# IceTTTb/NopeSAC

Measured on AMD Instinct MI355X. Metric: image-pairs/sec (480x640, K=32 hyp), higher is better.
Workload: dtype bf16; 1 GPU; configs/inference_mp3d.yaml, 32 synthetic 480x640 pairs/GPU/step, ResNet-50 + pyramids in bfloat16, head GEMMs bf16 operands with f32 accumulate / residual stream / LayerNorm / softmax, K=32 matched planes forced (m mean 32.0), nq=50; pairs_per_gpu=32, global_batch=32, K=32, parallelism=pair-sharded dp1, rccl_ranks=1, batches_in_flight_per_gpu=4, hip_graph=False, steps_per_all_gather=8, routing_entries_loaded=45, routing_entries_measured_now=0, nonfinite_outputs=0

## Files before the change

include/nopesac_hip.h:

```cpp
#ifndef NOPESAC_HIP_H
#define NOPESAC_HIP_H

#include <stdint.h>

#ifdef __cplusplus
extern "C" {
#endif

#define NPS_DT_F32 0
#define NPS_DT_BF16 1
#define NPS_DT_F32_BF16W 2
#define NPS_DT_FP8 3

#define NPS_ACT_NONE 0
#define NPS_ACT_RELU 1
#define NPS_ACT_LEAKY 2
#define NPS_ACT_SIGMOID 3
#define NPS_ACT_RES_AFTER 0x100
#define NPS_ACT_BIAS_BATCHED 0x200

#define NPS_E_ARG (-1)
#define NPS_E_UNSUPPORTED (-2)
typedef int nps_status;

// ... 248 lines not shown
nps_status nopesac_force_k_select(const float* logits, int n_cls, const float* query_feat, const int64_t* perm, const float* noise,
                                  int B, int nq, int K, int D, float* feats, int32_t* n_kept, void* stream);

nps_status nopesac_normalize_rows(const float* x, float* y, int rows, int D, int canonical_sign, void* stream);

nps_status nopesac_count_nonfinite(const float* x, int64_t n, int32_t* count, void* stream);
nps_status nopesac_u8_to_f32(const uint8_t* x, float* y, int64_t n, void* stream);

nps_status nopesac_clock_probe(uint64_t* out2, int64_t spin_cycles, void* stream);

#define NOPESAC_NONFINITE_MAX_TENSORS 16
nps_status nopesac_count_nonfinite_batch(const float* const* x, const int64_t* n, int n_tensors, int32_t* count, void* stream);

#define NOPESAC_JPEG_HUFF_BYTES 1536
#define NOPESAC_JPEG_TABLES_BYTES (4 * NOPESAC_JPEG_HUFF_BYTES + 3 * 128)
#define NOPESAC_JPEG_IMG_I32 32
#define NOPESAC_JPEG_IMG_I64 8
#define NOPESAC_JPEG_SEG_I32 4
#define NOPESAC_JPEG_SEG_I64 2
nps_status nopesac_jpeg_huffman(const int32_t* img32, const int64_t* img64, const uint8_t* tables, const int32_t* seg32, const int64_t* seg64,
                                int n_segments, const uint32_t* words, int64_t n_words, int16_t* coef, const int32_t* par_done, void* stream);
int64_t nopesac_jpeg_prepare_scan(const uint8_t* data, int64_t n, int has_restart, uint32_t* words, int64_t words_cap, int64_t* seg_off,
                                  int64_t* seg_cnt, int64_t* seg_bytes, int64_t max_segs, int64_t* consumed);
void* nopesac_jpeg_batch_scan_host(const char* const* paths, int n, int threads, int parallel, int* status, int64_t* totals);
int nopesac_jpeg_batch_fill_host(void* batch, int32_t* img32, int64_t* img64, uint8_t* tables, int32_t* seg32, int64_t* seg64, uint32_t* words,
                                 int32_t* lane_img, int32_t* geometry);
void nopesac_jpeg_batch_free_host(void* batch);
#define NOPESAC_JPEG_SUB_WORDS 64
#define NOPESAC_JPEG_SYNC_PASSES 12
nps_status nopesac_jpeg_huffman_parallel(const int32_t* img32, const int64_t* img64, const uint8_t* tables, int n_images, const int32_t* lane_img,
                                         int64_t n_lanes, const uint32_t* words, int64_t n_words, int64_t* exit_state, int64_t* entry_used,
                                         int32_t* n_blk, int64_t* first_block, int32_t* changed, int32_t* par_done, int16_t* coef, void* stream);
nps_status nopesac_jpeg_idct(const int32_t* img32, const int64_t* img64, const uint8_t* tables, int n_images, int n_blocks, const int16_t* coef,
                             uint8_t* planes, void* stream);
nps_status nopesac_jpeg_color(const int32_t* img32, const int64_t* img64, int n_images, int max_pixels, const uint8_t* planes, uint8_t* out,
                              int bgr, void* stream);

#define NOPESAC_GATHER_MAX_SEGMENTS 32
nps_status nopesac_gather_bytes(const void* const* src, const int64_t* size, const int64_t* const* size_dev, const int64_t* dst_off,
                                int n_segments, void* dst, void* stream);

nps_status nopesac_gnn_layer_bf16(const float* x, int x_off, const float* src, int src_off, float* out, int out_off, int n_sets, int nq,
                                  const int32_t* qlen, const int32_t* klen, const void* wq, const void* wk, const void* wv,
                                  const void* wmerge, const void* w0, const void* w2, const float* ln1_g, const float* ln1_b,
                                  const float* ln2_g, const float* ln2_b, void* stream);
nps_status nopesac_gnn_layer_bf16_pf(const float* x, int x_off, const float* src, int src_off, float* out, int out_off, int n_sets,
                                     int nq, const int32_t* qlen, const int32_t* klen, const void* wq, const void* wk, const void* wv,
                                     const void* wmerge, const void* w0, const void* w2, const float* ln1_g, const float* ln1_b,
                                     const float* ln2_g, const float* ln2_b, const void* const* next_weights6, int next_sets, void* stream);

nps_status nopesac_mask_head_bf16(const void* c1, const void* t1, const void* w_lateral, const float* scale, const float* bias,
                                  const void* mask_w, const float* mask_b, float* prob, void* p1_out, int B, int H, int W, int nq,
                                  int apply_sigmoid, void* stream);

nps_status nopesac_mask_operands(const float* fold, int ld, void* mask_w, float* mask_b, int B, int nq, int nqp, void* stream);

nps_status nopesac_encoder_tail_bf16(const void* attn, const float* src, const void* wo, const float* bo, const float* ln1_g,
                                     const float* ln1_b, const void* w1, const float* b1, const void* w2, const float* b2,
                                     const float* ln2_g, const float* ln2_b, const float* pos, int pos_rows, float* y, void* y_bf16,
                                     void* ypos_bf16, int M, void* stream);

nps_status nopesac_resize_bilinear_u8(const uint8_t* src, int H, int W, int C, uint8_t* dst, int OH, int OW, void* stream);
nps_status nopesac_resize_bilinear_u8_batch(const uint8_t* src, int n, int64_t src_stride, int H, int W, int C, uint8_t* dst, int OH, int OW, int chw,
                                            void* stream);

nps_status nopesac_decoder_tail_bf16(const void* attn, const float* tgt, const void* wo, const float* bo, const float* ln3_g,
                                     const float* ln3_b, const void* w1, const float* b1, const void* w2, const float* b2,
                                     const float* lnn_g, const float* lnn_b, const float* pos, int pos_rows, float* y, void* y_bf16,
                                     void* ypos_bf16, float* yn, int M, void* stream);

nps_status nopesac_transformer_tail_bf16(const void* attn, const float* src, const void* wo, const float* bo, const float* lna_g,
                                         const float* lna_b, const void* w1, const float* b1, const void* w2, const float* b2,
                                         const float* lnb_g, const float* lnb_b, const float* pos, int pos_rows, float* y, void* y_bf16,
                                         void* ypos_bf16, float* yn, int pre_norm, int skip_ffn, const void* w_pos, const float* b_pos,
                                         void* proj_pos, int n_pos, const void* w_proj, const float* b_proj, void* proj, int n_proj, int M,
                                         void* stream);
nps_status nopesac_transformer_tail_bf16_pf(const void* attn, const float* src, const void* wo, const float* bo, const float* lna_g,
                                            const float* lna_b, const void* w1, const float* b1, const void* w2, const float* b2,
                                            const float* lnb_g, const float* lnb_b, const float* pos, int pos_rows, float* y, void* y_bf16,
                                            void* ypos_bf16, float* yn, int pre_norm, int skip_ffn, const void* w_pos, const float* b_pos,
                                            void* proj_pos, int n_pos, const void* w_proj, const float* b_proj, void* proj, int n_proj, int M,
                                            const void* const* next_ptrs, const int64_t* next_bytes, int n_next, int next_workgroups, void* stream);

#define NPS_ETAIL_32 0
#define NPS_ETAIL_64 1
#define NPS_ETAIL_96 2
#define NPS_ETAIL_128 3
#define NPS_ETAIL_FORMS 4
#define NPS_ETAIL_SW_32 1
#define NPS_ETAIL_SW_64 2
#define NPS_ETAIL_SW_ROWS 4
#define NPS_ETAIL_SW_ROWS3 8
int nopesac_transformer_tail_forms(long long M, int pre_norm, int skip_ffn, long long n_proj_total, int switches, unsigned* eligible);
nps_status nopesac_transformer_tail_bf16_form(const void* attn, const float* src, const void* wo, const float* bo, const float* lna_g,
                                              const float* lna_b, const void* w1, const float* b1, const void* w2, const float* b2,
                                              const float* lnb_g, const float* lnb_b, const float* pos, int pos_rows, float* y, void* y_bf16,
                                              void* ypos_bf16, float* yn, int pre_norm, int skip_ffn, const void* w_pos, const float* b_pos,
                                              void* proj_pos, int n_pos, const void* w_proj, const float* b_proj, void* proj, int n_proj, int M,
                                              const void* const* next_ptrs, const int64_t* next_bytes, int n_next, int next_workgroups, int form,
                                              void* stream);

nps_status nopesac_rle_labels(const uint8_t* winner, const int32_t* kept_idx, const int32_t* n_kept, const int32_t* flags,
                              uint8_t* labels, int V, int H, int W, int nq, void* stream);
nps_status nopesac_rle_transitions(const uint8_t* labels, const int32_t* n_kept, const int64_t* offsets, int32_t* counts,
                                   uint32_t* positions, int V, int N, int nq, void* stream);
nps_status nopesac_decode_masks(const uint8_t* winner, const int32_t* kept_idx, const int32_t* n_kept, const int32_t* flags,
// ... 158 lines not shown
```

nopesac_amd/build.py:

```python
from __future__ import annotations

import hashlib
import os
import shutil
import subprocess
import sys
from concurrent.futures import ThreadPoolExecutor

HERE = os.path.dirname(os.path.abspath(__file__))
CSRC = os.path.join(HERE, "csrc")
LIB = os.path.join(HERE, "libnopesac_hip.so")
OBJ = os.path.join(CSRC, "_obj")
SOURCES = ["capi.hip", "conv_igemm.hip", "conv_p8.hip", "conv_p8n.hip", "stem.hip", "conv3x3_c64.hip", "conv3x3_halo.hip", "pwchain.hip", "gnn_layer.hip", "enc_tail.hip", "mask_head.hip", "resize.hip", "rle.hip", "plane_eval.hip", "elementwise.hip", "attention.hip", "postselect.hip", "matcher.hip",
           "ransac.hip", "refine_bwd.hip", "conv_bwd.hip", "matcher_bwd.hip", "plane_criterion.hip", "mlp_chain.hip", "tape.hip", "posenet_branch.hip", "jpeg.hip", "jpeg_host.hip", "png_host.hip"]
FLAGS = ["--offload-arch=gfx950", "-O3", "-std=c++17", "-fPIC", "-ffp-contract=off", "-Xclang", "-target-feature", "-Xclang", "-packed-fp32-ops"]
if os.environ.get("NOPESAC_ALLOW_PACKED_FP32"):
    FLAGS = FLAGS[:5]
EXTRA_FLAGS = {}
if os.environ.get("NOPESAC_HIPCC_EXTRA"):
    FLAGS = FLAGS + os.environ["NOPESAC_HIPCC_EXTRA"].split()


def _hipcc() -> str:
    for c in (os.environ.get("HIPCC"), shutil.which("hipcc"), "/opt/rocm/bin/hipcc"):
        if c and os.path.exists(c):
            return c
    raise RuntimeError("hipcc not found (need ROCm with gfx950 support)")


def _have_zlib(cc: str) -> bool:
    import tempfile
    with tempfile.TemporaryDirectory() as d:
        src = os.path.join(d, "z.cpp")
        with open(src, "w") as f:
            f.write("#include <zlib.h>\nint main() { z_stream s{}; return inflateInit(&s) == Z_OK ? inflateEnd(&s) : 1; }\n")
        r = subprocess.run([cc, "-x", "c++", src, "-o", os.path.join(d, "z"), "-lz"], capture_output=True, text=True)
        return r.returncode == 0


def _digest() -> str:
    h = hashlib.sha256((" ".join(FLAGS) + repr(sorted(EXTRA_FLAGS.items()))).encode())
    for name in sorted(os.listdir(CSRC)) + ["../../include/nopesac_hip.h"]:
        p = os.path.join(CSRC, name)
        if os.path.isfile(p) and (name.endswith((".hip", ".h"))):
            h.update(name.encode())
            h.update(open(p, "rb").read())
    return h.hexdigest()


def build(force: bool = False, verbose: bool = True) -> str:
    stamp = os.path.join(OBJ, "digest.txt")
    dig = _digest()
    if not force and os.path.exists(LIB) and os.path.exists(stamp) and open(stamp).read() == dig:
        return LIB
    os.makedirs(OBJ, exist_ok=True)
    cc = _hipcc()
    have_zlib = _have_zlib(cc)
    per_build = {"png_host.hip": ["-DNPS_HAVE_ZLIB=%d" % int(have_zlib)]}

    def compile_one(src):
        obj = os.path.join(OBJ, src.replace(".hip", ".o"))
        cmd = [cc, *FLAGS, *EXTRA_FLAGS.get(src, []), *per_build.get(src, []), "-c", os.path.join(CSRC, src), "-o", obj]
        r = subprocess.run(cmd, capture_output=True, text=True)
        if r.returncode != 0:
            raise RuntimeError("hipcc failed on %s:\n%s" % (src, r.stderr[-4000:]))
        return obj
# ... 17 lines not shown
```

nopesac_amd/csrc/common.h:

```cpp
#pragma once
#include <hip/hip_runtime.h>
#include <stdint.h>
#include <stdio.h>
#include <string.h>

#include <atomic>

#include "../../include/nopesac_hip.h"

namespace nps {

typedef unsigned short bf16_t;

__device__ __forceinline__ float bf16_to_f32(bf16_t v) { return __uint_as_float(((uint32_t)v) << 16); }
__device__ __forceinline__ bf16_t f32_to_bf16(float f) { return __builtin_bit_cast(bf16_t, (__bf16)f); }
__device__ __forceinline__ uint32_t f32x2_to_bf16x2(float lo, float hi) {
    typedef float f32x2_t __attribute__((ext_vector_type(2)));
    typedef __bf16 bf16x2_t __attribute__((ext_vector_type(2)));
    const f32x2_t v = {lo, hi};
    return __builtin_bit_cast(uint32_t, __builtin_convertvector(v, bf16x2_t));
}

__device__ __forceinline__ uint2 f32x8_to_fp8(const float* v) {
    float c[8];
// ... 5 lines not shown
    hi = __builtin_amdgcn_cvt_pk_fp8_f32(c[4], c[5], hi, false);
    hi = __builtin_amdgcn_cvt_pk_fp8_f32(c[6], c[7], hi, true);
    return make_uint2((unsigned)lo, (unsigned)hi);
}

template <typename T> __device__ __forceinline__ float to_f32(T v);
template <> __device__ __forceinline__ float to_f32<float>(float v) { return v; }
template <> __device__ __forceinline__ float to_f32<bf16_t>(bf16_t v) { return bf16_to_f32(v); }
template <typename T> __device__ __forceinline__ T from_f32(float v);
template <> __device__ __forceinline__ float from_f32<float>(float v) { return v; }
template <> __device__ __forceinline__ bf16_t from_f32<bf16_t>(float v) { return f32_to_bf16(v); }

__device__ __forceinline__ float apply_act(float v, int act) {
    if (act == NPS_ACT_SIGMOID) return 1.f / (1.f + expf(-v));
    const float neg = act == NPS_ACT_RELU ? 0.f : (act == NPS_ACT_LEAKY ? 0.01f * v : v);
    return v > 0.f ? v : neg;
}

template <int N>
__device__ __forceinline__ void apply_act_n(float (&v)[N], int act) {
    if (act == NPS_ACT_RELU) {
#pragma unroll
        for (int e = 0; e < N; ++e) v[e] = v[e] > 0.f ? v[e] : 0.f;
    } else if (act == NPS_ACT_LEAKY) {
#pragma unroll
        for (int e = 0; e < N; ++e) v[e] = v[e] > 0.f ? v[e] : 0.01f * v[e];
    } else if (act == NPS_ACT_SIGMOID) {
#pragma unroll
        for (int e = 0; e < N; ++e) v[e] = 1.f / (1.f + expf(-v[e]));
    }
}

__device__ __forceinline__ void act_residual8(float (&v)[8], const float (&r)[8], int act, int res_after) {
    if (!res_after) {
#pragma unroll
        for (int e = 0; e < 8; ++e) v[e] += r[e];
    }
    if (act == NPS_ACT_RELU) {
#pragma unroll
        for (int e = 0; e < 8; ++e) v[e] = v[e] > 0.f ? v[e] : 0.f;
    } else if (act == NPS_ACT_LEAKY) {
#pragma unroll
        for (int e = 0; e < 8; ++e) v[e] = v[e] > 0.f ? v[e] : 0.01f * v[e];
    } else if (act == NPS_ACT_SIGMOID) {
#pragma unroll
        for (int e = 0; e < 8; ++e) v[e] = 1.f / (1.f + expf(-v[e]));
    }
    if (res_after) {
#pragma unroll
        for (int e = 0; e < 8; ++e) v[e] += r[e];
    }
}

__device__ __forceinline__ float wave_sum(float v) {
#pragma unroll
    for (int o = 32; o > 0; o >>= 1) v += __shfl_xor(v, o, 64);
    return v;
}
__device__ __forceinline__ float wave_max(float v) {
#pragma unroll
    for (int o = 32; o > 0; o >>= 1) v = fmaxf(v, __shfl_xor(v, o, 64));
    return v;
}

__device__ __forceinline__ void quat_to_rot(const float q[4], float R[9]) {
    const float w = q[0], x = q[1], y = q[2], z = q[3];
    R[0] = 1 - 2 * y * y - 2 * z * z; R[1] = 2 * x * y - 2 * w * z; R[2] = 2 * x * z + 2 * w * y;
    R[3] = 2 * x * y + 2 * w * z; R[4] = 1 - 2 * x * x - 2 * z * z; R[5] = 2 * y * z - 2 * w * x;
    R[6] = 2 * x * z - 2 * w * y; R[7] = 2 * y * z + 2 * w * x; R[8] = 1 - 2 * x * x - 2 * y * y;
}

__device__ __forceinline__ void warp_plane(const float p[3], const float R[9], const float t[3], float out[3]) {
    const float f0 = p[0], f1 = -p[1], f2 = -p[2];
    float e[3], b[3];
#pragma unroll
    for (int i = 0; i < 3; ++i) {
        float s = __fmul_rn(R[3 * i], f0);
        s = __fmaf_rn(R[3 * i + 1], f1, s);
        s = __fmaf_rn(R[3 * i + 2], f2, s);
        e[i] = __fadd_rn(s, t[i]);
        b[i] = __fsub_rn(e[i], t[i]);
    }
    const float dot = e[0] * b[0] + e[1] * b[1] + e[2] * b[2];
    const float nb = sqrtf(b[0] * b[0] + b[1] * b[1] + b[2] * b[2]) + 1e-5f;
    const float c = dot / (nb * nb);
    out[0] = c * b[0]; out[1] = c * b[1]; out[2] = c * b[2];
}

__device__ __forceinline__ float norm3(const float v[3]) { return sqrtf(v[0] * v[0] + v[1] * v[1] + v[2] * v[2]); }
__device__ __forceinline__ void normalize3(const float v[3], float o[3]) {
    const float n = fmaxf(norm3(v), 1e-12f);
    o[0] = v[0] / n; o[1] = v[1] / n; o[2] = v[2] / n;
}

void set_error(const char* fmt, ...);

}

#define NPS_CHECK_ARG(cond, ...)               \
    do {                                       \
        if (!(cond)) {                         \
            nps::set_error(__VA_ARGS__);       \
            return NPS_E_ARG;                  \
        }                                      \
    } while (0)

// ... 22 lines not shown
```

nopesac_amd/csrc/elementwise.hip:

```cpp
#include <algorithm>

#include "common.h"

namespace nps {

template <typename T>
__global__ void preprocess_kernel(const float* __restrict__ x, T* __restrict__ y, const float* __restrict__ mean,
                                  const float* __restrict__ stdv, int B, int C, int H, int W, int Cpad) {
    const long long npix = (long long)B * H * W;
    for (long long i = blockIdx.x * (long long)blockDim.x + threadIdx.x; i < npix; i += (long long)gridDim.x * blockDim.x) {
        const long long b = i / ((long long)H * W), hw = i % ((long long)H * W);
        for (int c = 0; c < Cpad; ++c) {
            float v = 0.f;
            if (c < C) v = (x[(b * C + c) * H * W + hw] - mean[c]) / stdv[c];
            y[i * Cpad + c] = from_f32<T>(v);
        }
    }
}

template <typename T, int V> struct Pack { T v[V]; };
template <typename T, int V> __device__ __forceinline__ void load_vec(const T* p, float out[V]) {
    if constexpr (V == 1) { out[0] = to_f32<T>(*p); }
    else {
        typedef Pack<T, V> __attribute__((aligned(sizeof(T) * V))) PV;
// ... 5 lines not shown
template <typename T, int V> __device__ __forceinline__ void store_vec(T* p, const float in[V]) {
    if constexpr (V == 1) { *p = from_f32<T>(in[0]); }
    else {
        typedef Pack<T, V> __attribute__((aligned(sizeof(T) * V))) PV;
        PV pk;
#pragma unroll
        for (int i = 0; i < V; ++i) pk.v[i] = from_f32<T>(in[i]);
        *reinterpret_cast<PV*>(p) = pk;
    }
}

template <typename T, int V>
__global__ void maxpool_kernel(const T* __restrict__ x, T* __restrict__ y, int B, int H, int W, int C, int K,
                               int stride, int pad, int OH, int OW) {
    const int CV = C / V;
    const long long total = (long long)B * OH * OW * CV;
    for (long long i = blockIdx.x * (long long)blockDim.x + threadIdx.x; i < total; i += (long long)gridDim.x * blockDim.x) {
        const int c = (int)(i % CV) * V;
        long long pix = i / CV;
        const int ow = pix % OW; pix /= OW;
        const int oh = pix % OH;
        const int b = pix / OH;
        float m[V];
#pragma unroll
        for (int e = 0; e < V; ++e) m[e] = -INFINITY;
        for (int kh = 0; kh < K; ++kh) {
            const int ih = oh * stride - pad + kh;
            if ((unsigned)ih >= (unsigned)H) continue;
            for (int kw = 0; kw < K; ++kw) {
                const int iw = ow * stride - pad + kw;
                if ((unsigned)iw >= (unsigned)W) continue;
                float t[V];
                load_vec<T, V>(x + (((long long)b * H + ih) * W + iw) * C + c, t);
#pragma unroll
                for (int e = 0; e < V; ++e) m[e] = fmaxf(m[e], t[e]);
            }
        }
        store_vec<T, V>(y + (i / CV) * C + c, m);
    }
}

template <typename T, int V>
__global__ void upsample_bilinear2x_kernel(const T* __restrict__ x, const T* __restrict__ addend, T* __restrict__ y,
                                           int B, int H, int W, int C, int act) {
    const int OH = 2 * H, OW = 2 * W, CV = C / V;
    const long long total = (long long)B * OH * OW * CV;
    for (long long i = blockIdx.x * (long long)blockDim.x + threadIdx.x; i < total; i += (long long)gridDim.x * blockDim.x) {
        const int c = (int)(i % CV) * V;
        long long pix = i / CV;
        const long long opix = pix;
        const int ow = pix % OW; pix /= OW;
        const int oh = pix % OH;
        const int b = pix / OH;
        float sy = fmaxf(0.5f * (oh + 0.5f) - 0.5f, 0.f), sx = fmaxf(0.5f * (ow + 0.5f) - 0.5f, 0.f);
        const int y0 = (int)sy, x0 = (int)sx;
        const int y1 = min(y0 + 1, H - 1), x1 = min(x0 + 1, W - 1);
        const float ly = sy - y0, lx = sx - x0, hy = 1.f - ly, hx = 1.f - lx;
        const long long base = (long long)b * H * W;
        float v00[V], v01[V], v10[V], v11[V], o[V];
        load_vec<T, V>(x + (base + (long long)y0 * W + x0) * C + c, v00);
        load_vec<T, V>(x + (base + (long long)y0 * W + x1) * C + c, v01);
        load_vec<T, V>(x + (base + (long long)y1 * W + x0) * C + c, v10);
        load_vec<T, V>(x + (base + (long long)y1 * W + x1) * C + c, v11);
#pragma unroll
        for (int e = 0; e < V; ++e) o[e] = hy * (hx * v00[e] + lx * v01[e]) + ly * (hx * v10[e] + lx * v11[e]);
        apply_act_n<V>(o, act);
        if (addend) {
            float a[V];
            load_vec<T, V>(addend + opix * C + c, a);
#pragma unroll
            for (int e = 0; e < V; ++e) o[e] += a[e];
        }
        store_vec<T, V>(y + opix * C + c, o);
    }
}

template <typename T, int V>
__global__ void upsample_nearest2x_add_kernel(const T* __restrict__ x, const T* __restrict__ lat, T* __restrict__ y,
                                              int B, int H, int W, int C) {
    const int OH = 2 * H, OW = 2 * W, CV = C / V;
    const long long total = (long long)B * OH * OW * CV;
    for (long long i = blockIdx.x * (long long)blockDim.x + threadIdx.x; i < total; i += (long long)gridDim.x * blockDim.x) {
        const int c = (int)(i % CV) * V;
        long long pix = i / CV;
        const long long opix = pix;
        const int ow = pix % OW; pix /= OW;
        const int oh = pix % OH;
        const int b = pix / OH;
        float a[V], l[V];
        load_vec<T, V>(x + (((long long)b * H + (oh >> 1)) * W + (ow >> 1)) * C + c, a);
        load_vec<T, V>(lat + opix * C + c, l);
#pragma unroll
        for (int e = 0; e < V; ++e) a[e] += l[e];
        store_vec<T, V>(y + opix * C + c, a);
    }
}

template <typename T>
__global__ __launch_bounds__(256) void groupnorm_kernel(const T* __restrict__ x, const float* __restrict__ gamma,
                                                        const float* __restrict__ beta, T* __restrict__ y, int HW,
                                                        int C, int G, float eps, int act, int groups_per_block) {
    const int cpg = C / G;
    const int CPB = cpg * groups_per_block;
    const int b = blockIdx.y, chunk = blockIdx.x;
    const int c_local = threadIdx.x % CPB, prow = threadIdx.x / CPB, nprow = 256 / CPB;
    const int c = chunk * CPB + c_local;
    const int g_local = c_local / cpg;
    const T* xb = x + (long long)b * HW * C;
    T* yb = y + (long long)b * HW * C;
    __shared__ float red[256];
    __shared__ float stat[64];
    const float cnt = (float)HW * cpg;
    float s = 0.f;
    for (int p = prow; p < HW; p += nprow) s += to_f32<T>(xb[(long long)p * C + c]);
    red[threadIdx.x] = s;
    __syncthreads();
    if (threadIdx.x < groups_per_block) {
        float t = 0.f;
// ... 649 lines not shown
```

nopesac_amd/modeling/plane_head.py:

```python
from __future__ import annotations

import os

import math

import torch

from .. import _lib, ops
from ..registry import SEM_SEG_HEADS_REGISTRY
from ..synth import state_dict_spec
from .params import ConvW, ParamModule, conv_bias, conv_bn, mlp_layers


def sine_position_embedding(h: int, w: int, num_pos_feats: int = 128) -> torch.Tensor:
    eps, scale, temperature = 1e-6, 2 * math.pi, 10000.0
    y = torch.arange(1, h + 1, dtype=torch.float32).view(h, 1).expand(h, w)
    x = torch.arange(1, w + 1, dtype=torch.float32).view(1, w).expand(h, w)
    y = y / (y[-1:, :] + eps) * scale
    x = x / (x[:, -1:] + eps) * scale
    dim_t = torch.arange(num_pos_feats, dtype=torch.float32)
    dim_t = temperature ** (2 * torch.div(dim_t, 2, rounding_mode="floor") / num_pos_feats)
    px, py = x[:, :, None] / dim_t, y[:, :, None] / dim_t
    px = torch.stack((px[..., 0::2].sin(), px[..., 1::2].cos()), dim=3).flatten(2)
    py = torch.stack((py[..., 0::2].sin(), py[..., 1::2].cos()), dim=3).flatten(2)
# ... 19 lines not shown
    flat, last_of, restarts = [], [], []
    for si, (layers, final_act, out) in enumerate(stacks):
        for i, l in enumerate(layers):
            last = i == len(layers) - 1
            flat.append((l, final_act if last else ops.ACT_RELU))
            last_of.append(si if last else -1)
            restarts.append(par[si] and si > 0 and i == 0)
    want = [o for (_, _, o) in stacks]
    for si in range(len(stacks)):
        if want[si] is None and (si == len(stacks) - 1 or par[si + 1]):
            want[si] = True
    results = [None] * len(stacks)
    for si, o in enumerate(want):
        if o is True:
            results[si] = torch.empty(rows, stacks[si][0][-1].cout, device=x.device, dtype=torch.float32)
        elif o is not None:
            results[si] = o
    k0 = x.shape[1] + (0 if x_bcast is None else x_bcast.shape[1])
    few_rows = rows <= CHAIN_MIN_ROWS and sum(l.cout * l.cin for l, _ in flat) >= CHAIN_SMALL_PARAMS
    if (gd == torch.bfloat16 and x.dtype == torch.float32 and len(flat) <= _lib.MLP_MAX_LAYERS and k0 <= _lib.MLP_MAX_IN
            and all(l.cout <= _lib.MLP_MAX_WIDTH for l, _ in flat) and not few_rows):
        ops.mlp_chain(x, [l.chain() for l, _ in flat], [a for _, a in flat], [results[si] if si >= 0 else None for si in last_of],
                      x_bcast=x_bcast, rows_per=rows_per, restarts=restarts)
        return results
    if x_bcast is not None:
        assert rows == x_bcast.shape[0] * rows_per, "run_stacks: x_bcast rows x rows_per must equal the rows of x"
        full = torch.empty(rows, k0, device=x.device, dtype=torch.float32)
        full.view(-1, rows_per, k0)[:, :, :x_bcast.shape[1]] = x_bcast[:, None, :]
        full[:, x_bcast.shape[1]:] = x
        x = full
    x_in = x
    for (l, a), si, rs in zip(flat, last_of, restarts):
        inner = gd == torch.bfloat16 and (si < 0 or results[si] is None)
        x = ops.linear(x_in if rs else x, l.w2d(gd), l.bias, act=a, out=results[si] if si >= 0 else None,
                       out_dtype=torch.bfloat16 if inner else None)
    return results


@SEM_SEG_HEADS_REGISTRY.register()
class PlaneTRHead(ParamModule):
    def __init__(self, cfg, input_shape=None):
        H = cfg.MODEL.SEM_SEG_HEAD
        self.num_queries = H.NUM_OBJECT_QUERIES
        self.nheads = H.NHEADS
        assert H.HIDDEN_DIM == 256 and H.MASK_DIM == 256 and H.NHEADS == 8 and H.ENC_LAYERS == 6 and H.DEC_LAYERS == 6, \
            "PlaneTRHead kernels are specialised to hidden 256 / 8 heads / 6+6 layers (config/config.py:46-51)"
        assert H.PARAM_ON and H.CENTER_ON and not cfg.MODEL.DEPTH_ON, "inference configs set PARAM_ON/CENTER_ON, no depth"
        spec = {k[len("sem_seg_head."):]: v for k, v in state_dict_spec(self.num_queries).items()
                if k.startswith("sem_seg_head.")}
        super().__init__(spec)
        self._pos_cache = {}
        self.fused_encoder_tail = True
        self.fused_mask_head = True
        self.fused_decoder_tail = True
        self.chain_projections = True

    def _mha(self, prefix: str, fuse_qk: bool):
        w, b = self.raw(prefix + ".in_proj_weight").float(), self.raw(prefix + ".in_proj_bias").float()
        E = 256
        d = {"o": conv_bias(self, prefix + ".out_proj"), "v": ConvW(w[2 * E:], None, b[2 * E:])}
        if fuse_qk:
            d["qk"] = ConvW(w[:2 * E], None, b[:2 * E])
        else:
            d["q"], d["k"] = ConvW(w[:E], None, b[:E]), ConvW(w[E:2 * E], None, b[E:2 * E])
        return d

    def pack(self) -> dict:
        P = {"input_proj": conv_bias(self, "input_proj")}
        for i in range(6):
            p = f"context_SA.layers.{i}"
            P[p] = {"attn": self._mha(p + ".self_attn", True), "l1": conv_bias(self, p + ".linear1"),
                    "l2": conv_bias(self, p + ".linear2")}
            p = f"context2plane_decoder.layers.{i}"
            P[p] = {"self": self._mha(p + ".self_attn", True), "cross": self._mha(p + ".multihead_attn", False),
                    "l1": conv_bias(self, p + ".linear1"), "l2": conv_bias(self, p + ".linear2")}
        wk = [self.raw(f"context2plane_decoder.layers.{i}.multihead_attn.in_proj_weight").float()[256:512] for i in range(6)]
        bk = [self.raw(f"context2plane_decoder.layers.{i}.multihead_attn.in_proj_bias").float()[256:512] for i in range(6)]
        wv = [self.raw(f"context2plane_decoder.layers.{i}.multihead_attn.in_proj_weight").float()[512:768] for i in range(6)]
        bv = [self.raw(f"context2plane_decoder.layers.{i}.multihead_attn.in_proj_bias").float()[512:768] for i in range(6)]
        P["cross_k_all"] = ConvW(torch.cat(wk, 0), None, torch.cat(bk, 0))
        P["cross_v_all"] = ConvW(torch.cat(wv, 0), None, torch.cat(bv, 0))
        for nm in ("up_conv3", "up_conv2", "up_conv1", "c4_conv", "c3_conv", "c2_conv", "c1_conv", "m_conv_dict.m4"):
            P[nm] = conv_bn(self, f"top_down.{nm}.0.weight", f"top_down.{nm}.1", 1e-5)
        for nm in ("plane_embedding", "plane_param", "plane_center"):
            P[nm] = mlp_layers(self, nm)
        P["pixel_embedding"] = conv_bias(self, "pixel_embedding")
        w_pe = self.raw("pixel_embedding.weight").float().reshape(256, 256)
        fold = torch.zeros(264, 256, device=w_pe.device)
        fold[:256] = w_pe.t()
        fold[256] = self.raw("pixel_embedding.bias").float()
        P["pe_fold"] = ConvW(fold)
        P["pixel_plane_center"] = conv_bias(self, "pixel_plane_center")
        P["plane_prob"] = conv_bias(self, "plane_prob")
        return P

    def _ln(self, x, prefix, **kw):
        return ops.layernorm(x, self.raw(prefix + ".weight"), self.raw(prefix + ".bias"), **kw)

    def _pos(self, h, w, device):
        key = (h, w, str(device))
        if key not in self._pos_cache:
            self._pos_cache[key] = sine_position_embedding(h, w).to(device)
        return self._pos_cache[key]

    def forward(self, features: dict, want_logits: bool = False):
        P, gd = self.packed, self.gemm_dtype
# ... 157 lines not shown
                    hs = r["yn"]
                continue
            tgt = lin(o, W["cross"]["o"].w2d(bf), W["cross"]["o"].bias, residual=tgt, out_dtype=f32)
            r = ln(tgt, p + ".norm3", want=("y16",))
            hdn = lin(r["y16"], W["l1"].w2d(bf), W["l1"].bias, act=ops.ACT_RELU, out_dtype=bf)
            tgt = lin(hdn, W["l2"].w2d(bf), W["l2"].bias, residual=tgt, out_dtype=f32)
            if i < 5:
                nin = ln(tgt, nxt, addend=qpos, want=("y16", "y2_16"))
                n16, npos16 = nin["y16"], nin["y2_16"]
        if hs is None:
            hs = self._ln(tgt, "context2plane_decoder.norm")
        return hs, memory

    def _tail_weights(self, kind: str, i: int) -> dict:
        cache = self.__dict__.setdefault("_tail_w", {})
        if (kind, i) not in cache:
            bf = torch.bfloat16
            f = lambda k: self.raw(k).float().contiguous()
            if kind == "enc":
                e = self._enc_tail_weights(i)
                cache[(kind, i)] = dict(e, ga=e["g1"], bea=e["be1"], gb=e["g2"], beb=e["be2"])
            elif kind == "dec":
                d = self._dec_tail_weights(i, f"context2plane_decoder.layers.{i + 1}.norm1" if i < 5 else "context2plane_decoder.norm")
                cache[(kind, i)] = dict(d, ga=d["g3"], bea=d["be3"], gb=d["gn"], beb=d["ben"])
            else:
                p, W = f"context2plane_decoder.layers.{i}", self.packed[f"context2plane_decoder.layers.{i}"]
                cache[(kind, i)] = {"wo": W["self"]["o"].wfrag(bf), "bo": W["self"]["o"].bias, "ga": f(p + ".norm2.weight"), "bea": f(p + ".norm2.bias")}
        return cache[(kind, i)]

    def _dec_tail_weights(self, i: int, next_norm: str) -> dict:
        cache = self.__dict__.setdefault("_dec_tail_w", {})
        if i not in cache:
            p, W = f"context2plane_decoder.layers.{i}", self.packed[f"context2plane_decoder.layers.{i}"]
            f = lambda k: self.raw(k).float().contiguous()
            cache[i] = {"wo": W["cross"]["o"].wfrag(torch.bfloat16), "bo": W["cross"]["o"].bias, "w1": W["l1"].wfrag(torch.bfloat16),
                        "b1": W["l1"].bias, "w2": W["l2"].wfrag(torch.bfloat16), "b2": W["l2"].bias,
                        "g3": f(p + ".norm3.weight"), "be3": f(p + ".norm3.bias"),
                        "gn": f(next_norm + ".weight"), "ben": f(next_norm + ".bias")}
        return cache[i]

    def _heads(self, features, hs, memory, B, hc, wc, nq, want_logits, mark):
        P, gd = self.packed, self.gemm_dtype
        c1, c2, c3, c4 = features["res2"], features["res3"], features["res4"], features["res5"]
        cd = c4.dtype
        RA = ops.ACT_RELU | ops.ACT_RES_AFTER

        def cbr(x, nm, residual=None, out_dtype=None):
            c = P[nm]
            return ops.conv2d(x, c.w(gd if x.dtype == torch.float32 else x.dtype), c.scale, c.bias, residual,
                              act=RA if residual is not None else ops.ACT_RELU, out_dtype=out_dtype)

        p4 = cbr(memory.view(B, hc, wc, 256), "m_conv_dict.m4", residual=cbr(c4, "c4_conv"), out_dtype=cd)

        def up_stage(x, nm, lateral):
            c = P[nm]
            t = ops.conv2d(x, c.w(x.dtype), c.scale, c.bias, act=ops.ACT_NONE)
            return ops.upsample2x_bilinear(t, lateral, act=ops.ACT_RELU)

        p3 = up_stage(p4, "up_conv3", cbr(c3, "c3_conv"))
        p2 = up_stage(p3, "up_conv2", cbr(c2, "c2_conv"))
        if gd == torch.bfloat16 and hs.dtype == torch.float32:
            r = run_stacks(hs, [(P["plane_embedding"], ops.ACT_NONE, None), ([P["pe_fold"]], ops.ACT_NONE, True),
                                ([P["plane_prob"]], ops.ACT_NONE, True), (P["plane_param"], ops.ACT_NONE, True),
                                (P["plane_center"], ops.ACT_SIGMOID, True)], gd, parallel=[False, False, True, True, True])
            fold = r[1]
            heads = {"pred_logits": r[2].view(B, nq, 2), "pred_params": r[3].view(B, nq, 3), "pred_centers": r[4].view(B, nq, 2)}
        else:
            fold = run_stacks(hs, [(P["plane_embedding"], ops.ACT_NONE, None), ([P["pe_fold"]], ops.ACT_NONE, True)], gd)[1]
            heads = {
                "pred_logits": run_mlp(hs, [P["plane_prob"]], gd=gd).view(B, nq, 2),
                "pred_params": run_mlp(hs, P["plane_param"], gd=gd).view(B, nq, 3),
                "pred_centers": run_mlp(hs, P["plane_center"], final_act=ops.ACT_SIGMOID, gd=gd).view(B, nq, 2),
            }
        h1, w1 = c1.shape[1], c1.shape[2]
        if (self.fused_mask_head and cd == torch.bfloat16 and not want_logits and nq <= 128 and nq % 2 == 0 and (h1 * w1) % 128 == 0):
            c = P["up_conv1"]
            t1 = ops.conv2d(p2, c.w(cd), c.scale, c.bias, act=ops.ACT_NONE)
            l = P["c1_conv"]
            mark("ph.top_down")
            heads["mask_prob"] = ops.mask_head(c1, t1, l.wfrag(cd), l.scale, l.bias, None, None, fold=fold)
            return heads, hs.view(B, nq, 256)
        p1 = up_stage(p2, "up_conv1", cbr(c1, "c1_conv"))
        mark("ph.top_down")
        mw = fold[:, :256].to(cd).contiguous().view(B, nq, 1, 1, 256)
        mb = fold[:, 256].contiguous().view(B, nq)
        out = dict(heads)
        out["mask_prob"] = ops.conv2d(p1, mw, None, mb, batched_weights=True, act=ops.ACT_SIGMOID, out_dtype=torch.float32)
        if want_logits:
            out["pred_mask_logits"] = ops.conv2d(p1, mw, None, mb, batched_weights=True, out_dtype=torch.float32)
            pc = P["pixel_plane_center"]
            out["pixel_centers"] = ops.conv2d(p1, pc.w(cd), None, pc.bias, act=ops.ACT_SIGMOID, out_dtype=torch.float32)
        return out, hs.view(B, nq, 256)


def build_planeTR_head(cfg, input_shape=None):
    return SEM_SEG_HEADS_REGISTRY.get(cfg.MODEL.SEM_SEG_HEAD.NAME)(cfg, input_shape)


def post_select(head_out: dict, query_feat: torch.Tensor, height: int, width: int, cfg) -> dict:
    return ops.postselect_planes(head_out["pred_logits"], head_out["mask_prob"], head_out["pred_params"], query_feat,
                                 height, width, float(cfg.TEST.PLANE_SCORE_THRESHOLD), float(cfg.TEST.MASK_PROB_THRESHOLD),
                                 float(cfg.TEST.OVERLAP_THRESHOLD), planar=bool(head_out.get("mask_prob_planar", False)))
```

nopesac_amd/ops.py:

```python
from __future__ import annotations

from collections import namedtuple
from typing import Optional

import ctypes
import functools
import os

import torch

from . import _lib

_H = _lib.H
F32, BF16, FP8 = _H.NPS_DT_F32, _H.NPS_DT_BF16, _H.NPS_DT_FP8
ACT_NONE, ACT_RELU, ACT_LEAKY, ACT_SIGMOID = _H.NPS_ACT_NONE, _H.NPS_ACT_RELU, _H.NPS_ACT_LEAKY, _H.NPS_ACT_SIGMOID
ACT_RES_AFTER = _H.NPS_ACT_RES_AFTER
ACT_BIAS_BATCHED = _H.NPS_ACT_BIAS_BATCHED
_DT = {torch.float32: F32, torch.bfloat16: BF16, torch.float8_e4m3fn: FP8}


class OpsArgumentError(AssertionError, ValueError):
    """A wrapper's argument check failed.  Raised explicitly (not `assert`): the checks stay in force under `python -O`.
    (Subclasses AssertionError so that callers written against the first version keep working.)"""

# ... 1060 lines not shown


def resize_bilinear_u8(img: torch.Tensor, out_h: int, out_w: int) -> torch.Tensor:
    _chk(img, torch.uint8)
    H, W, C = img.shape
    out = torch.empty((out_h, out_w, C), device=img.device, dtype=torch.uint8)
    _C.nopesac_resize_bilinear_u8(_p(img), H, W, C, _p(out), out_h, out_w, _stream())
    return out


def resize_bilinear_u8_batch(imgs, out_h: int, out_w: int, chw: bool = True) -> torch.Tensor:
    a = imgs[0]
    _chk(a, torch.uint8)
    H, W, C = a.shape
    n = len(imgs)
    stride = (imgs[1].data_ptr() - a.data_ptr()) if n > 1 else H * W * C
    st = a.untyped_storage().data_ptr()
    if stride < H * W * C or any(im.shape != a.shape or not im.is_contiguous() or im.data_ptr() != a.data_ptr() + k * stride
                                 or im.untyped_storage().data_ptr() != st for k, im in enumerate(imgs)):
        return None
    out = torch.empty((n, C, out_h, out_w) if chw else (n, out_h, out_w, C), device=a.device, dtype=torch.uint8)
    _C.nopesac_resize_bilinear_u8_batch(_p(a), n, stride, H, W, C, _p(out), out_h, out_w, 1 if chw else 0, _stream())
    return out


def mask_head(c1: torch.Tensor, t1: torch.Tensor, w_lat_frag: torch.Tensor, scale, bias, mask_w: torch.Tensor, mask_b: torch.Tensor,
              sigmoid: bool = True, want_p1: bool = False, planar: bool = False, fold: Optional[torch.Tensor] = None, taps1: bool = False,
              pipe: bool = False):
    _chk(c1, torch.bfloat16); _chk(t1, torch.bfloat16); _chk(w_lat_frag, torch.bfloat16)
    B, H, W, C = c1.shape
    nq = mask_w.shape[1] if fold is None else fold.shape[0] // B
    _require(C == 256 and t1.shape == (B, H // 2, W // 2, 256) and nq <= 128 and nq % 2 == 0 and (H * W) % 128 == 0,
             'mask_head: C == 256, t1 at half resolution, nq even and <= 128, H * W a multiple of 128')
    nqp = 64 if nq <= 64 else 128
    if fold is not None:
        _chk(fold, torch.float32)
        _require(fold.dim() == 2 and fold.shape[0] == B * nq and fold.shape[1] >= 257 and fold.is_contiguous(), "mask_head: fold [B * nq, >= 257]")
        mw = torch.empty(B, nqp // 32, 16, 2, 32, 8, device=c1.device, dtype=torch.bfloat16)
        mb = torch.empty(B, nqp, device=c1.device, dtype=torch.float32)
        _C.nopesac_mask_operands(_p(fold), fold.shape[1], _p(mw), _p(mb), B, nq, nqp, _stream())
    else:
        mw = torch.zeros(B, nqp, 256, device=c1.device, dtype=torch.bfloat16)
        mw[:, :nq] = mask_w
        mw = mw.view(B, nqp // 32, 32, 16, 2, 8).permute(0, 1, 3, 4, 2, 5).contiguous()
        mb = torch.zeros(B, nqp, device=c1.device, dtype=torch.float32)
        mb[:, :nq] = mask_b
    prob = torch.empty((B, nq, H, W) if planar else (B, H, W, nq), device=c1.device, dtype=torch.float32)
    p1 = torch.empty(B, H, W, 256, device=c1.device, dtype=torch.bfloat16) if want_p1 else None
    _C.nopesac_mask_head_bf16(_p(c1), _p(t1), _p(w_lat_frag), _p(scale), _p(bias), _p(mw), _p(mb), _p(prob), _p(p1), B, H, W, nq,
                              int(sigmoid) | (2 if planar else 0) | (4 if taps1 else 0) | (8 if pipe else 0), _stream())
    return (prob, p1) if want_p1 else prob


def decoder_tail(attn: torch.Tensor, tgt: torch.Tensor, W: dict, pos=None, want=("y", "y16", "ypos16")) -> dict:
    _chk(attn, torch.bfloat16); _chk(tgt, torch.float32)
    M = tgt.shape[0]
    _require(attn.shape == (M, 256) and tgt.shape == (M, 256), 'argument check failed: attn.shape == (M, 256) and tgt.shape == (M, 256)')
    out = {k: torch.empty(M, 256, device=tgt.device, dtype=torch.float32 if k in ("y", "yn") else torch.bfloat16) for k in want}
    if pos is not None:
        _chk(pos, torch.float32)
    _C.nopesac_decoder_tail_bf16(_p(attn), _p(tgt), _p(W["wo"]), _p(W["bo"]), _p(W["g3"]), _p(W["be3"]), _p(W["w1"]), _p(W["b1"]),
                                 _p(W["w2"]), _p(W["b2"]), _p(W["gn"]), _p(W["ben"]), _p(pos), 0 if pos is None else pos.shape[0],
                                 _p(out.get("y")), _p(out.get("y16")), _p(out.get("ypos16")), _p(out.get("yn")), M, _stream())
    return out


TAIL_PREFETCH = os.environ.get("NOPESAC_TAIL_PREFETCH", "1") != "0"
TRANSFORMER_TAIL_FORMS = _forms_by_id({"t32": _H.NPS_ETAIL_32, "t64": _H.NPS_ETAIL_64, "t96": _H.NPS_ETAIL_96, "t128": _H.NPS_ETAIL_128}, _H.NPS_ETAIL_FORMS)
TRANSFORMER_TAIL_SWITCHES = {"NOPESAC_ENC_TAIL_32": _H.NPS_ETAIL_SW_32, "NOPESAC_ENC_TAIL_64": _H.NPS_ETAIL_SW_64,
                             "NOPESAC_ENC_TAIL_ROWS": _H.NPS_ETAIL_SW_ROWS, "NOPESAC_ENC_TAIL_ROWS=3": _H.NPS_ETAIL_SW_ROWS3}


def transformer_tail_forms(M, pre_norm, skip_ffn=False, n_proj_total=0, switches=0):
    mask = ctypes.c_uint(0)
    form = _C.nopesac_transformer_tail_forms(M, int(bool(pre_norm)), int(bool(skip_ffn)), n_proj_total, switches, ctypes.byref(mask))
    return form, mask.value


def transformer_tail(attn: torch.Tensor, src: torch.Tensor, W: dict, *, pre_norm: bool, skip_ffn: bool = False, pos=None,
                     want=("y",), proj_pos=None, proj=None, prefetch=None, form=None, out=None) -> dict:
    _chk(attn, torch.bfloat16); _chk(src, torch.float32)
    M = src.shape[0]
    _require(attn.shape == (M, 256) and src.shape == (M, 256), "transformer_tail: attn / src [M, 256]")
    given = dict(out or {})
    if pos is not None:
        _chk(pos, torch.float32)
    wa, ba, na = proj_pos if proj_pos is not None else (None, None, 0)
    wb, bb, nb = proj if proj is not None else (None, None, 0)
    shapes = {k: (256, torch.float32 if k in ("y", "yn") else torch.bfloat16) for k in want}
    if na:
        shapes["proj_pos"] = (na, torch.bfloat16)
    if nb:
        shapes["proj"] = (nb, torch.bfloat16)
    _require(set(given) <= set(shapes), "transformer_tail: out holds a buffer that was not asked for")
    out = {}
    for k, (n, dt) in shapes.items():
        t = given.get(k)
        if t is None:
            t = torch.empty(M, n, device=src.device, dtype=dt)
        _chk(t, dt)
        _require(t.shape == (M, n), "transformer_tail: out[%s] must be [M, %d]" % (k, n))
        out[k] = t
    g = W.get
    nptr = nbytes = None
    n_next = next_wg = 0
    if prefetch is not None and TAIL_PREFETCH and M <= 64 * 32:
# ... 306 lines not shown
```

Measured before the change: 4066 pairs/s.

## Fuse FPN top-down upsample, lateral add and next 1x1 conv into one kernel

Adds a HIP kernel that bilinearly upsamples the low-resolution top-down feature by 2x, applies ReLU, adds the lateral, and then immediately runs the next stage's 1x1 conv (MFMA bf16 GEMM with scale/bias) on the LDS-resident tile. This removes the intermediate p3/p2 tensors' round trips to global memory and two kernel launches per stage in the plane head. The fused path is on by default for bf16. It adds a specialised kernel with a 4-pixel shared-column load path, at the cost of more LDS use and some risk in tile-boundary handling.

New measurement: 4102 pairs/s, median of 6. Within noise of the previous version (+0.9%).

```diff
diff --git a/include/nopesac_hip.h b/include/nopesac_hip.h
--- a/include/nopesac_hip.h
+++ b/include/nopesac_hip.h
@@ -324,6 +324,9 @@
 nps_status nopesac_mask_head_bf16(const void* c1, const void* t1, const void* w_lateral, const float* scale, const float* bias,
                                   const void* mask_w, const float* mask_b, float* prob, void* p1_out, int B, int H, int W, int nq,
                                   int apply_sigmoid, void* stream);
+
+nps_status nopesac_topdown_up_bf16(const void* t_low, const void* lateral, const void* w_up, const float* scale, const float* bias,
+                                   void* y, void* p_out, int B, int H, int W, void* stream);
 
 nps_status nopesac_mask_operands(const float* fold, int ld, void* mask_w, float* mask_b, int B, int nq, int nqp, void* stream);
 
diff --git a/nopesac_amd/build.py b/nopesac_amd/build.py
--- a/nopesac_amd/build.py
+++ b/nopesac_amd/build.py
@@ -11,7 +11,7 @@
 CSRC = os.path.join(HERE, "csrc")
 LIB = os.path.join(HERE, "libnopesac_hip.so")
 OBJ = os.path.join(CSRC, "_obj")
-SOURCES = ["capi.hip", "conv_igemm.hip", "conv_p8.hip", "conv_p8n.hip", "stem.hip", "conv3x3_c64.hip", "conv3x3_halo.hip", "pwchain.hip", "gnn_layer.hip", "enc_tail.hip", "mask_head.hip", "resize.hip", "rle.hip", "plane_eval.hip", "elementwise.hip", "attention.hip", "postselect.hip", "matcher.hip",
+SOURCES = ["capi.hip", "conv_igemm.hip", "conv_p8.hip", "conv_p8n.hip", "stem.hip", "conv3x3_c64.hip", "conv3x3_halo.hip", "pwchain.hip", "gnn_layer.hip", "enc_tail.hip", "mask_head.hip", "topdown_up.hip", "resize.hip", "rle.hip", "plane_eval.hip", "elementwise.hip", "attention.hip", "postselect.hip", "matcher.hip",
            "ransac.hip", "refine_bwd.hip", "conv_bwd.hip", "matcher_bwd.hip", "plane_criterion.hip", "mlp_chain.hip", "tape.hip", "posenet_branch.hip", "jpeg.hip", "jpeg_host.hip", "png_host.hip"]
 FLAGS = ["--offload-arch=gfx950", "-O3", "-std=c++17", "-fPIC", "-ffp-contract=off", "-Xclang", "-target-feature", "-Xclang", "-packed-fp32-ops"]
 if os.environ.get("NOPESAC_ALLOW_PACKED_FP32"):
diff --git a/nopesac_amd/csrc/common.h b/nopesac_amd/csrc/common.h
--- a/nopesac_amd/csrc/common.h
+++ b/nopesac_amd/csrc/common.h
@@ -81,6 +81,12 @@
     }
 }
 
+__device__ __forceinline__ float bilinear2x_src(int o) { return fmaxf(0.5f * (o + 0.5f) - 0.5f, 0.f); }
+__device__ __forceinline__ float bilinear2x_blend(float v00, float v01, float v10, float v11, float lx, float ly) {
+    const float hy = 1.f - ly, hx = 1.f - lx;
+    return hy * (hx * v00 + lx * v01) + ly * (hx * v10 + lx * v11);
+}
+
 __device__ __forceinline__ float wave_sum(float v) {
 #pragma unroll
     for (int o = 32; o > 0; o >>= 1) v += __shfl_xor(v, o, 64);
diff --git a/nopesac_amd/csrc/elementwise.hip b/nopesac_amd/csrc/elementwise.hip
--- a/nopesac_amd/csrc/elementwise.hip
+++ b/nopesac_amd/csrc/elementwise.hip
@@ -81,10 +81,10 @@
         const int ow = pix % OW; pix /= OW;
         const int oh = pix % OH;
         const int b = pix / OH;
-        float sy = fmaxf(0.5f * (oh + 0.5f) - 0.5f, 0.f), sx = fmaxf(0.5f * (ow + 0.5f) - 0.5f, 0.f);
+        const float sy = bilinear2x_src(oh), sx = bilinear2x_src(ow);
         const int y0 = (int)sy, x0 = (int)sx;
         const int y1 = min(y0 + 1, H - 1), x1 = min(x0 + 1, W - 1);
-        const float ly = sy - y0, lx = sx - x0, hy = 1.f - ly, hx = 1.f - lx;
+        const float ly = sy - y0, lx = sx - x0;
         const long long base = (long long)b * H * W;
         float v00[V], v01[V], v10[V], v11[V], o[V];
         load_vec<T, V>(x + (base + (long long)y0 * W + x0) * C + c, v00);
@@ -92,7 +92,7 @@
         load_vec<T, V>(x + (base + (long long)y1 * W + x0) * C + c, v10);
         load_vec<T, V>(x + (base + (long long)y1 * W + x1) * C + c, v11);
 #pragma unroll
-        for (int e = 0; e < V; ++e) o[e] = hy * (hx * v00[e] + lx * v01[e]) + ly * (hx * v10[e] + lx * v11[e]);
+        for (int e = 0; e < V; ++e) o[e] = bilinear2x_blend(v00[e], v01[e], v10[e], v11[e], lx, ly);
         apply_act_n<V>(o, act);
         if (addend) {
             float a[V];
diff --git a/nopesac_amd/csrc/topdown_up.hip b/nopesac_amd/csrc/topdown_up.hip
--- /dev/null
+++ b/nopesac_amd/csrc/topdown_up.hip
@@ -0,0 +1,169 @@
+#include "conv_common.h"
+
+namespace nps {
+
+constexpr int TU_C = 256, TU_LD = TU_C + 8, TU_BM = 128, TU_RT = TU_BM / 32, TU_RING = 8;
+constexpr size_t TU_TILE_BYTES = (size_t)(2 * TU_BM * TU_LD);
+constexpr size_t TU_LDS_TOTAL = TU_TILE_BYTES + 512 * sizeof(float);
+static_assert(2 * TU_LDS_TOTAL <= 160 * 1024, "two workgroups per CU");
+
+struct TopdownUpArgs {
+    const bf16_t* t; const bf16_t* lat;
+    const bf16_t* w; const float* sc; const float* bc;
+    bf16_t* y; bf16_t* p_out;
+    int B, H, W, M;
+};
+
+__global__ __launch_bounds__(512, 4) void topdown_up_kernel(const TopdownUpArgs p) {
+    extern __shared__ __attribute__((aligned(16))) unsigned char tu_smem[];
+    bf16_t* At = reinterpret_cast<bf16_t*>(tu_smem);
+    float* SB = reinterpret_cast<float*>(tu_smem + TU_TILE_BYTES);
+    const int tid = threadIdx.x, lane = tid & 63, l31 = lane & 31, half = lane >> 5;
+    const int wave = __builtin_amdgcn_readfirstlane(tid >> 6);
+    const int OW = 2 * p.W, per = 4 * p.H * p.W;
+    int bid = blockIdx.x;
+    {
+        const int nwg = gridDim.x, q = nwg / 8, r = nwg % 8, xcd = bid % 8, within = bid / 8;
+        bid = (xcd < r ? xcd * (q + 1) : r * (q + 1) + (xcd - r) * q) + within;
+    }
+    const int m0 = bid * TU_BM;
+
+    bf16x8 ring[TU_RING];
+    const bf16_t* wp = p.w + ((long long)wave * 16 * 64 + lane) * 8;
+    const float sb_s = p.sc[tid & 255], sb_b = p.bc[tid & 255];
+#pragma unroll
+    for (int s = 0; s < TU_RING; ++s) ring[s] = *reinterpret_cast<const bf16x8*>(wp + s * 512);
+#pragma unroll
+    for (int i = 0; i < TU_BM * 32 / 512; ++i) {
+        const int c = tid + i * 512, r = c >> 5, col = (c & 31) * 8;
+        const int m = min(m0 + r, p.M - 1);
+        *reinterpret_cast<us8*>(At + r * TU_LD + col) = *reinterpret_cast<const us8*>(p.lat + (long long)m * TU_C + col);
+    }
+    if (tid < 256) { SB[tid] = sb_s; SB[256 + tid] = sb_b; }
+    NPS_LDS_SYNC();
+
+    {
+        typedef unsigned int u32x4_t __attribute__((ext_vector_type(4)));
+        auto lo = [](unsigned int wd) { return __uint_as_float(wd << 16); };
+        auto hi = [](unsigned int wd) { return __uint_as_float(wd & 0xffff0000u); };
+        auto blend_store = [&](int r, int col, const u32x4_t& v00, const u32x4_t& v01, const u32x4_t& v10, const u32x4_t& v11, float lx, float ly) {
+            const u32x4_t lw = *reinterpret_cast<const u32x4_t*>(At + r * TU_LD + col);
+            u32x4_t ow4;
+#pragma unroll
+            for (int e = 0; e < 4; ++e) {
+                float a = bilinear2x_blend(lo(v00[e]), lo(v01[e]), lo(v10[e]), lo(v11[e]), lx, ly);
+                float b = bilinear2x_blend(hi(v00[e]), hi(v01[e]), hi(v10[e]), hi(v11[e]), lx, ly);
+                a = (a > 0.f ? a : 0.f) + lo(lw[e]);
+                b = (b > 0.f ? b : 0.f) + hi(lw[e]);
+                ow4[e] = f32x2_to_bf16x2(a, b);
+            }
+            const us8 l8 = __builtin_bit_cast(us8, ow4);
+            *reinterpret_cast<us8*>(At + r * TU_LD + col) = l8;
+            if (p.p_out && m0 + r < p.M) *reinterpret_cast<us8*>(p.p_out + (long long)(m0 + r) * TU_C + col) = l8;
+        };
+        if ((OW & 3) == 0) {
+#pragma unroll 1
+            for (int i = 0; i < TU_BM * 8 / 512; ++i) {
+                const int c = tid + i * 512, r0 = (c >> 5) * 4, col = (c & 31) * 8;
+                const int m = min(m0 + r0, p.M - 4);
+                const int b = m / per, rem = m - b * per, oh = rem / OW, ow = rem - oh * OW;
+                const float sy = bilinear2x_src(oh);
+                const int y0 = (int)sy, y1 = min(y0 + 1, p.H - 1);
+                const float ly = sy - y0;
+                const int j2 = ow >> 1;
+                const int ca = max(j2 - 1, 0), cb = j2, cc = min(j2 + 1, p.W - 1), cd = min(j2 + 2, p.W - 1);
+                const bf16_t* r0p = p.t + (((long long)b * p.H + y0) * p.W) * TU_C + col;
+                const bf16_t* r1p = p.t + (((long long)b * p.H + y1) * p.W) * TU_C + col;
+                const u32x4_t a0 = *reinterpret_cast<const u32x4_t*>(r0p + ca * TU_C), b0 = *reinterpret_cast<const u32x4_t*>(r0p + cb * TU_C);
+                const u32x4_t c0 = *reinterpret_cast<const u32x4_t*>(r0p + cc * TU_C), d0 = *reinterpret_cast<const u32x4_t*>(r0p + cd * TU_C);
+                const u32x4_t a1 = *reinterpret_cast<const u32x4_t*>(r1p + ca * TU_C), b1 = *reinterpret_cast<const u32x4_t*>(r1p + cb * TU_C);
+                const u32x4_t c1 = *reinterpret_cast<const u32x4_t*>(r1p + cc * TU_C), d1 = *reinterpret_cast<const u32x4_t*>(r1p + cd * TU_C);
+                auto lx_of = [](int o) { const float sx = bilinear2x_src(o); return sx - (float)(int)sx; };
+                blend_store(r0, col, a0, b0, a1, b1, lx_of(ow), ly);
+                blend_store(r0 + 1, col, b0, c0, b1, c1, lx_of(ow + 1), ly);
+                blend_store(r0 + 2, col, b0, c0, b1, c1, lx_of(ow + 2), ly);
+                blend_store(r0 + 3, col, c0, d0, c1, d1, lx_of(ow + 3), ly);
+            }
+        } else {
+#pragma unroll 2
+            for (int i = 0; i < TU_BM * 32 / 512; ++i) {
+                const int c = tid + i * 512, r = c >> 5, col = (c & 31) * 8;
+                const int m = min(m0 + r, p.M - 1);
+                const int b = m / per, rem = m - b * per, oh = rem / OW, ow = rem - oh * OW;
+                const float sy = bilinear2x_src(oh), sx = bilinear2x_src(ow);
+                const int y0 = (int)sy, x0 = (int)sx, y1 = min(y0 + 1, p.H - 1), x1 = min(x0 + 1, p.W - 1);
+                const bf16_t* tb = p.t + (long long)b * p.H * p.W * TU_C + col;
+                const u32x4_t v00 = *reinterpret_cast<const u32x4_t*>(tb + ((long long)y0 * p.W + x0) * TU_C);
+                const u32x4_t v01 = *reinterpret_cast<const u32x4_t*>(tb + ((long long)y0 * p.W + x1) * TU_C);
+                const u32x4_t v10 = *reinterpret_cast<const u32x4_t*>(tb + ((long long)y1 * p.W + x0) * TU_C);
+                const u32x4_t v11 = *reinterpret_cast<const u32x4_t*>(tb + ((long long)y1 * p.W + x1) * TU_C);
+                blend_store(r, col, v00, v01, v10, v11, sx - x0, sy - y0);
+            }
+        }
+    }
+    NPS_LDS_SYNC();
+
+    {
+        f32x16 acc[TU_RT];
+#pragma unroll
+        for (int r = 0; r < TU_RT; ++r)
+#pragma unroll
+            for (int e = 0; e < 16; ++e) acc[r][e] = 0.f;
+#pragma unroll
+        for (int kk = 0; kk < 16; ++kk) {
+#pragma unroll
+            for (int r = 0; r < TU_RT; ++r) {
+                const bf16x8 af = *reinterpret_cast<const bf16x8*>(At + (r * 32 + l31) * TU_LD + kk * 16 + half * 8);
+                acc[r] = __builtin_amdgcn_mfma_f32_32x32x16_bf16(ring[kk % TU_RING], af, acc[r], 0, 0, 0);
+            }
+            if (kk + TU_RING < 16) ring[kk % TU_RING] = *reinterpret_cast<const bf16x8*>(wp + (kk + TU_RING) * 512);
+            if ((kk & 1) == 1) __builtin_amdgcn_sched_barrier(0);
+        }
+        NPS_LDS_SYNC();
+#pragma unroll
+        for (int q = 0; q < 4; ++q) {
+            const int n = wave * 32 + 8 * q + 4 * half;
+            const f32x4 s = *reinterpret_cast<const f32x4*>(SB + n), bb = *reinterpret_cast<const f32x4*>(SB + 256 + n);
+#pragma unroll
+            for (int r = 0; r < TU_RT; ++r) {
+                us4 o;
+#pragma unroll
+                for (int e = 0; e < 4; ++e) {
+                    float v = acc[r][4 * q + e] * s[e];
+                    v += bb[e];
+                    v += 0.f;
+                    o[e] = f32_to_bf16(v);
+                }
+                *reinterpret_cast<us4*>(At + (r * 32 + l31) * TU_LD + n) = o;
+            }
+        }
+    }
+    NPS_LDS_SYNC();
+    int tl = tid;
+    asm volatile("" : "+v"(tl));
+#pragma unroll
+    for (int i = 0; i < TU_BM * 32 / 512; ++i) {
+        const int c = tl + i * 512, r = c >> 5, col = (c & 31) * 8;
+        const us8 v = *reinterpret_cast<const us8*>(At + r * TU_LD + col);
+        if (m0 + r < p.M) *reinterpret_cast<us8*>(p.y + (long long)(m0 + r) * TU_C + col) = v;
+    }
+}
+
+}
+
+extern "C" int nopesac_topdown_up_bf16(const void* t_low, const void* lateral, const void* w_up, const float* scale, const float* bias,
+                                       void* y, void* p_out, int B, int H, int W, void* stream) {
+    using namespace nps;
+    NPS_CHECK_ARG(t_low && lateral && w_up && scale && bias && y, "topdown_up: null pointer");
+    NPS_CHECK_ARG(B >= 1 && H >= 1 && W >= 1, "topdown_up: B, H, W must be >= 1");
+    const void* ptrs[] = {t_low, lateral, w_up, scale, bias, y, p_out};
+    for (const void* q : ptrs) NPS_CHECK_ARG(((uintptr_t)q & 15) == 0, "topdown_up: pointers must be 16-byte aligned");
+    const long long M = (long long)B * 4 * H * W;
+    NPS_CHECK_ARG(M < (1ll << 31) - TU_BM, "topdown_up: B * 2H * 2W must stay below 2^31");
+    TopdownUpArgs a;
+    a.t = (const bf16_t*)t_low; a.lat = (const bf16_t*)lateral; a.w = (const bf16_t*)w_up; a.sc = scale; a.bc = bias;
+    a.y = (bf16_t*)y; a.p_out = (bf16_t*)p_out; a.B = B; a.H = H; a.W = W; a.M = (int)M;
+    NPS_ENSURE_LDS((int)TU_LDS_TOTAL, topdown_up_kernel);
+    hipLaunchKernelGGL(topdown_up_kernel, dim3((unsigned)((M + TU_BM - 1) / TU_BM)), dim3(512), TU_LDS_TOTAL, (hipStream_t)stream, a);
+    NPS_LAUNCH_RET();
+}
diff --git a/nopesac_amd/modeling/plane_head.py b/nopesac_amd/modeling/plane_head.py
--- a/nopesac_amd/modeling/plane_head.py
+++ b/nopesac_amd/modeling/plane_head.py
@@ -95,6 +95,7 @@
         self._pos_cache = {}
         self.fused_encoder_tail = True
         self.fused_mask_head = True
+        self.fused_topdown = True
         self.fused_decoder_tail = True
         self.chain_projections = True
 
@@ -358,13 +359,25 @@
 
         p4 = cbr(memory.view(B, hc, wc, 256), "m_conv_dict.m4", residual=cbr(c4, "c4_conv"), out_dtype=cd)
 
+        def up_conv(x, nm):
+            c = P[nm]
+            return ops.conv2d(x, c.w(x.dtype), c.scale, c.bias, act=ops.ACT_NONE)
+
         def up_stage(x, nm, lateral):
+            return ops.upsample2x_bilinear(up_conv(x, nm), lateral, act=ops.ACT_RELU)
+
+        def up_fused(t, lateral, nm):
             c = P[nm]
-            t = ops.conv2d(x, c.w(x.dtype), c.scale, c.bias, act=ops.ACT_NONE)
-            return ops.upsample2x_bilinear(t, lateral, act=ops.ACT_RELU)
-
-        p3 = up_stage(p4, "up_conv3", cbr(c3, "c3_conv"))
-        p2 = up_stage(p3, "up_conv2", cbr(c2, "c2_conv"))
+            return ops.topdown_up(t, lateral, c.wfrag(cd), c.scale, c.bias)
+
+        fused_td = self.fused_topdown and cd == torch.bfloat16
+        if fused_td:
+            t2 = up_fused(up_conv(p4, "up_conv3"), cbr(c3, "c3_conv"), "up_conv2")
+            t1 = up_fused(t2, cbr(c2, "c2_conv"), "up_conv1")
+        else:
+            p3 = up_stage(p4, "up_conv3", cbr(c3, "c3_conv"))
+            p2 = up_stage(p3, "up_conv2", cbr(c2, "c2_conv"))
+            t1 = None
         if gd == torch.bfloat16 and hs.dtype == torch.float32:
             r = run_stacks(hs, [(P["plane_embedding"], ops.ACT_NONE, None), ([P["pe_fold"]], ops.ACT_NONE, True),
                                 ([P["plane_prob"]], ops.ACT_NONE, True), (P["plane_param"], ops.ACT_NONE, True),
@@ -380,13 +393,13 @@
             }
         h1, w1 = c1.shape[1], c1.shape[2]
         if (self.fused_mask_head and cd == torch.bfloat16 and not want_logits and nq <= 128 and nq % 2 == 0 and (h1 * w1) % 128 == 0):
-            c = P["up_conv1"]
-            t1 = ops.conv2d(p2, c.w(cd), c.scale, c.bias, act=ops.ACT_NONE)
+            if t1 is None:
+                t1 = up_conv(p2, "up_conv1")
             l = P["c1_conv"]
             mark("ph.top_down")
             heads["mask_prob"] = ops.mask_head(c1, t1, l.wfrag(cd), l.scale, l.bias, None, None, fold=fold)
             return heads, hs.view(B, nq, 256)
-        p1 = up_stage(p2, "up_conv1", cbr(c1, "c1_conv"))
+        p1 = up_stage(p2, "up_conv1", cbr(c1, "c1_conv")) if t1 is None else ops.upsample2x_bilinear(t1, cbr(c1, "c1_conv"), act=ops.ACT_RELU)
         mark("ph.top_down")
         mw = fold[:, :256].to(cd).contiguous().view(B, nq, 1, 1, 256)
         mb = fold[:, 256].contiguous().view(B, nq)
diff --git a/nopesac_amd/ops.py b/nopesac_amd/ops.py
--- a/nopesac_amd/ops.py
+++ b/nopesac_amd/ops.py
@@ -1136,6 +1136,17 @@
     return (prob, p1) if want_p1 else prob
 
 
+def topdown_up(t_low: torch.Tensor, lateral: torch.Tensor, w_frag: torch.Tensor, scale: torch.Tensor, bias: torch.Tensor, want_p: bool = False):
+    _chk(t_low, torch.bfloat16); _chk(lateral, torch.bfloat16); _chk(w_frag, torch.bfloat16); _chk(scale, torch.float32); _chk(bias, torch.float32)
+    B, H, W, C = t_low.shape
+    _require(C == 256 and lateral.shape == (B, 2 * H, 2 * W, 256) and w_frag.shape == (256, 256) and scale.numel() == 256 and bias.numel() == 256,
+             'topdown_up: 256 channels, lateral at twice the resolution of t_low, w_frag [256, 256], scale / bias [256]')
+    y = torch.empty_like(lateral)
+    p = torch.empty_like(lateral) if want_p else None
+    _C.nopesac_topdown_up_bf16(_p(t_low), _p(lateral), _p(w_frag), _p(scale), _p(bias), _p(y), _p(p), B, H, W, _stream())
+    return (y, p) if want_p else y
+
+
 def decoder_tail(attn: torch.Tensor, tgt: torch.Tensor, W: dict, pos=None, want=("y", "y16", "ypos16")) -> dict:
     _chk(attn, torch.bfloat16); _chk(tgt, torch.float32)
     M = tgt.shape[0]
```
